# mit-han-lab/qserve

Hardware: NVIDIA H100
Metric: tokens/s Llama-3-8B W4A8KV4 decode b64 (higher is better)
Workload: dtype s8

## Files before the change

qserve_b200/csrc/gemm.cu:

```cuda
#include <cstdarg>
#include <cstdio>
#include <cstdlib>
#include <cstring>
#include <mutex>
#include <unordered_map>

#include "common.cuh"
#include "launch.cuh"

namespace qs {

namespace {

constexpr int kBM = 128;
constexpr int kBK = 128;
constexpr int kSub = 2;
constexpr int kConsumers = 128;
constexpr int kNumThreads = 192;
constexpr int kFrag = 4;

enum { kModeW4Chn = 0, kModeW4Grp = 1, kModeW8 = 2 };

struct GemmParams {
  const uint8_t* s2_scales;
  const uint8_t* s2_zeros;
  const __half* wscales;
  const __half* w_szs;
  const __half* ascales;
  const __half* a_ssums;
  __half* out;
  int32_t* acc_out;
  int M, N, K;
  int m_tiles, kb_per_tile, split;
  unsigned long long* prof;
};

template <int MODE, int NT, int WS, int AS>
struct Cfg {
  static constexpr int kActSub = NT * kBK;
  static constexpr int kWSub = (MODE == kModeW8) ? kBM * kBK : kBM * kBK / 2;
  static constexpr int kS2Sub = (MODE == kModeW4Grp) ? 2 * kBM : 0;
  static constexpr int kActBytes = kSub * kActSub;
  static constexpr int kWBytes = kSub * kWSub;
  static constexpr int kS2Bytes = kSub * kS2Sub;
  static constexpr int kWStageTx = kWBytes + kS2Bytes;
  static constexpr int kOffAct = 0;
  static constexpr int kOffW = kOffAct + AS * kActBytes;
  static constexpr int kOffS2 = kOffW + WS * kWBytes;
  static constexpr int kPipeBytes = kOffS2 + WS * kS2Bytes;
  static constexpr int kRedBytes = NT * kBM * 4;
  static constexpr int kOffRow = (kPipeBytes > kRedBytes ? kPipeBytes : kRedBytes);
  static constexpr int kOffBar = kOffRow + 2 * NT * 4;
  static constexpr int kNumBars = 2 * WS + 2 * AS;
  static constexpr int kSmemBytes = kOffBar + kNumBars * 8;
  static constexpr int kCtasPerSm = (NT <= 64 && kSmemBytes <= 113 * 1024) ? 2 : 1;
  static_assert(kSmemBytes <= 227 * 1024, "shared memory overflow");
};

__device__ __forceinline__ unsigned long long gtime() {
  unsigned long long t;
  asm volatile("mov.u64 %0, %globaltimer;" : "=l"(t)::"memory");
  return t;
}
#define QS_PROF(slot) do { if (p.prof) p.prof[blockIdx.x * 16 + (slot)] = gtime(); } while (0)

__device__ __forceinline__ uint32_t cluster_ctarank() {
  uint32_t r;
  asm volatile("mov.u32 %0, %%cluster_ctarank;" : "=r"(r));
  return r;
}
__device__ __forceinline__ void cluster_sync_all() {
  asm volatile("barrier.cluster.arrive.release.aligned;\n\tbarrier.cluster.wait.acquire.aligned;" ::: "memory");
}
__device__ __forceinline__ void cluster_arrive() { asm volatile("barrier.cluster.arrive.release;" ::: "memory"); }
__device__ __forceinline__ void cluster_wait() { asm volatile("barrier.cluster.wait.acquire;" ::: "memory"); }
__device__ __forceinline__ uint32_t smid() {
  uint32_t r;
  asm volatile("mov.u32 %0, %%smid;" : "=r"(r));
  return r;
}
__device__ __forceinline__ uint32_t map_to_cta(uint32_t smem_addr, uint32_t rank) {
  uint32_t r;
  asm volatile("mapa.shared::cluster.u32 %0, %1, %2;" : "=r"(r) : "r"(smem_addr), "r"(rank));
  return r;
}
__device__ __forceinline__ void st_dsmem_u32(uint32_t addr, uint32_t v) {
  asm volatile("st.shared::cluster.u32 [%0], %1;" ::"r"(addr), "r"(v) : "memory");
}

template <int V>
struct IntTag { static constexpr int value = V; };

template <int MODE>
__device__ __forceinline__ float epilogue_one(int32_t acc, float ws, float wsz, float as, float asum) {
  float ps = __int2float_rn(acc);
  if constexpr (MODE == kModeW4Chn) {
    float t = __fmul_rn(__fmul_rn(ps, ws), as);
    float u = __fmul_rn(wsz, asum);
    return __fsub_rn(t, u);
  } else {
    return __fmul_rn(ps, __fmul_rn(ws, as));
  }
}

template <int MODE>
__device__ __forceinline__ int acc_channel(int h, int w, int r) {
  return (MODE == kModeW8) ? 64 * h + 16 * w + r : 32 * w + 16 * h + r;
}

template <int MODE, int NT, int WS, int AS, bool ACC>
__global__ void __launch_bounds__(kNumThreads, Cfg<MODE, NT, WS, AS>::kCtasPerSm)
gemm_kernel(const __grid_constant__ CUtensorMap tmap_act, const __grid_constant__ CUtensorMap tmap_w, const GemmParams p) {
  using C = Cfg<MODE, NT, WS, AS>;
  extern __shared__ __align__(1024) uint8_t smem[];
  if (threadIdx.x == 0 && (smem_u32(smem) & 1023u) != 0) __trap();
  uint8_t* s_act = smem + C::kOffAct;
  uint8_t* s_w = smem + C::kOffW;
  uint8_t* s_s2 = smem + C::kOffS2;
  int32_t* s_red = reinterpret_cast<int32_t*>(smem);
  float* s_asc = reinterpret_cast<float*>(smem + C::kOffRow);
  float* s_asum = s_asc + NT;
  uint64_t* bar_wfull = reinterpret_cast<uint64_t*>(smem + C::kOffBar);
  uint64_t* bar_wempty = bar_wfull + WS;
  uint64_t* bar_xfull = bar_wempty + WS;
  uint64_t* bar_xempty = bar_xfull + AS;

  const int warp = threadIdx.x >> 5;
  const int lane = threadIdx.x & 31;
  const int S = p.split;
  const int rank = (S > 1) ? static_cast<int>(cluster_ctarank()) : 0;
  const int tile = blockIdx.x / S;
  const int m_tile = tile % p.m_tiles, n_tile = tile / p.m_tiles;
  const int KB = p.kb_per_tile;
  const int kb_begin = (KB * rank) / S, kb_end = (KB * (rank + 1)) / S;
  const int n_kb = kb_end - kb_begin;
  if (threadIdx.x == 0) {
    QS_PROF(0);
    if (p.prof) p.prof[blockIdx.x * 16 + 15] = smid();
  }
  qs_trace(QS_K_GEMM, 0);

  if (threadIdx.x == 0) {
    tma_prefetch_desc(&tmap_act);
    tma_prefetch_desc(&tmap_w);
    for (int i = 0; i < WS; ++i) {
      mbar_init(&bar_wfull[i], 1);
      mbar_init(&bar_wempty[i], 4);
    }
    for (int i = 0; i < AS; ++i) {
      mbar_init(&bar_xfull[i], 1);
      mbar_init(&bar_xempty[i], 4);
    }
    fence_barrier_init();
  }
  __syncthreads();
  if (threadIdx.x == 0) { pdl_launch_dependents(); QS_PROF(1); }

  if (warp == 4) {
    if (lane == 0) {
      const int w_row = (MODE == kModeW8) ? n_tile * kBM : n_tile * 4;
      const uint8_t* s2s = p.s2_scales + static_cast<size_t>(n_tile) * kBM;
      const uint8_t* s2z = p.s2_zeros + static_cast<size_t>(n_tile) * kBM;
      int s = 0;
      uint32_t ph = 0;
      for (int it = 0; it < n_kb; ++it) {
        if (it >= WS) mbar_wait_nocall(&bar_wempty[s], ph);
        mbar_expect_tx(&bar_wfull[s], C::kWStageTx);
#pragma unroll
        for (int u = 0; u < kSub; ++u) {
          const int kb = (kb_begin + it) * kSub + u;
          tma_load_2d(s_w + s * C::kWBytes + u * C::kWSub, &tmap_w, (MODE == kModeW8) ? kb * kBK : kb * 256, w_row, &bar_wfull[s]);
          if constexpr (MODE == kModeW4Grp) {
            const int kg = kb < p.K / kBK ? kb : p.K / kBK - 1;
            bulk_copy_g2s(s_s2 + s * C::kS2Bytes + u * C::kS2Sub, s2s + static_cast<size_t>(kg) * p.N, kBM, &bar_wfull[s]);
            bulk_copy_g2s(s_s2 + s * C::kS2Bytes + u * C::kS2Sub + kBM, s2z + static_cast<size_t>(kg) * p.N, kBM, &bar_wfull[s]);
          }
        }
        if (++s == WS) { s = 0; if (it >= WS) ph ^= 1; }
      }
      QS_PROF(3);
    }
  } else if (warp == 5) {
    if (lane == 0) {
      const int a_row = m_tile * NT;
      pdl_wait();
      QS_PROF(2);
      qs_trace(QS_K_GEMM, 1, 5 * 32);
      int s = 0;
      uint32_t ph = 0;
      for (int it = 0; it < n_kb; ++it) {
        if (it >= AS) mbar_wait_nocall(&bar_xempty[s], ph);
        mbar_expect_tx(&bar_xfull[s], C::kActBytes);
#pragma unroll
        for (int u = 0; u < kSub; ++u)
          tma_load_2d(s_act + s * C::kActBytes + u * C::kActSub, &tmap_act, ((kb_begin + it) * kSub + u) * kBK, a_row, &bar_xfull[s]);
        if (++s == AS) { s = 0; if (it >= AS) ph ^= 1; }
      }
    }
  } else {
    int32_t acc[2][NT / 2];
#pragma unroll
    for (int h = 0; h < 2; ++h)
#pragma unroll
      for (int i = 0; i < NT / 2; ++i) acc[h][i] = 0;
    mbar_wait_nocall(&bar_wfull[0], 0);
    mbar_wait_nocall(&bar_xfull[0], 0);
    if (threadIdx.x == 0) QS_PROF(4);
    const bool leader = lane == 0;
    int sw = 0, sx = 0, prev_sw = WS - 1, prev_sx = AS - 1;
    uint32_t phw = 0, phx = 0;
    for (int it = 0; it < n_kb; ++it) {
      mbar_wait_nocall(&bar_wfull[sw], phw);
      mbar_wait_nocall(&bar_xfull[sx], phx);
      if constexpr (MODE == kModeW8) {
#pragma unroll
        for (int u = 0; u < kSub; ++u) {
          const uint64_t bdesc = gmma_desc_sw128(smem_u32(s_act + sx * C::kActBytes + u * C::kActSub));
          const uint64_t adesc = gmma_desc_sw128(smem_u32(s_w + sw * C::kWBytes + u * C::kWSub));
          wgmma_fence();
#pragma unroll
          for (int t = 0; t < kBK / 32; ++t) {
            wgmma_s8_ss(acc[0], adesc + t * 2, bdesc + t * 2);
            wgmma_s8_ss(acc[1], adesc + (64 * kBK >> 4) + t * 2, bdesc + t * 2);
          }
          wgmma_commit();
        }
        wgmma_wait<kSub>();
        mbar_arrive_if(&bar_wempty[prev_sw], it > 0 && leader);
        mbar_arrive_if(&bar_xempty[prev_sx], it > 0 && leader);
      } else {
        uint32_t fr[kFrag][2][4];
#pragma unroll
        for (int u = 0; u < kSub; ++u) {
          const uint64_t bdesc = gmma_desc_sw128(smem_u32(s_act + sx * C::kActBytes + u * C::kActSub));
          const uint8_t* wsrc = s_w + sw * C::kWBytes + u * C::kWSub + warp * 2048 + lane * 16;
          uint32_t sc4 = 0, zp4 = 0;
          if constexpr (MODE == kModeW4Grp) {
            const uint8_t* s2 = s_s2 + sw * C::kS2Bytes + u * C::kS2Sub + warp * 32 + (lane >> 2) * 4;
            sc4 = *reinterpret_cast<const uint32_t*>(s2);
            zp4 = *reinterpret_cast<const uint32_t*>(s2 + kBM);
          }
#pragma unroll
          for (int t = 0; t < 4; ++t) {
            const int j = u * 4 + t;
            const uint4 v = *reinterpret_cast<const uint4*>(wsrc + t * 512);
            uint32_t xl = v.x & 0x0F0F0F0Fu, xh = (v.x >> 4) & 0x0F0F0F0Fu;
            uint32_t yl = v.y & 0x0F0F0F0Fu, yh = (v.y >> 4) & 0x0F0F0F0Fu;
            uint32_t zl = v.z & 0x0F0F0F0Fu, zh = (v.z >> 4) & 0x0F0F0F0Fu;
            uint32_t wl = v.w & 0x0F0F0F0Fu, wh = (v.w >> 4) & 0x0F0F0F0Fu;
            if constexpr (MODE == kModeW4Grp) {
              const uint32_t s0 = sc4 & 0xFF, s1 = (sc4 >> 8) & 0xFF, s2 = (sc4 >> 16) & 0xFF, s3 = sc4 >> 24;
              const uint32_t z0 = __byte_perm(zp4, 0, 0x0000), z1 = __byte_perm(zp4, 0, 0x1111);
              const uint32_t z2 = __byte_perm(zp4, 0, 0x2222), z3 = __byte_perm(zp4, 0, 0x3333);
              xl = __vadd4(xl * s0, z0); zl = __vadd4(zl * s0, z0);
              yl = __vadd4(yl * s1, z1); wl = __vadd4(wl * s1, z1);
              xh = __vadd4(xh * s2, z2); zh = __vadd4(zh * s2, z2);
              yh = __vadd4(yh * s3, z3); wh = __vadd4(wh * s3, z3);
            }
            wgmma_wait<kFrag - 1>();
            if (j == kFrag - 1) mbar_arrive_if(&bar_xempty[prev_sx], it > 0 && leader);
            uint32_t(&f)[2][4] = fr[j % kFrag];
            f[0][0] = xl; f[0][1] = yl; f[0][2] = zl; f[0][3] = wl;
            f[1][0] = xh; f[1][1] = yh; f[1][2] = zh; f[1][3] = wh;
            wgmma_fence();
            wgmma_s8_rs(acc[0], f[0], bdesc + t * 2);
            wgmma_s8_rs(acc[1], f[1], bdesc + t * 2);
            wgmma_commit();
          }
        }
        mbar_arrive_if(&bar_wempty[sw], leader);
      }
      prev_sw = sw;
      prev_sx = sx;
      if (++sw == WS) { sw = 0; phw ^= 1; }
      if (++sx == AS) { sx = 0; phx ^= 1; }
    }
    wgmma_wait<0>();
    if (threadIdx.x == 0) QS_PROF(6);
    if (S > 1) cluster_arrive();

    const int epi_tid = threadIdx.x;
    pdl_wait();
    const int m0 = m_tile * NT;
    for (int j = epi_tid; j < NT; j += kConsumers) {
      const bool ok = (m0 + j) < p.M;
      s_asc[j] = ok ? __half2float(p.ascales[m0 + j]) : 0.f;
      if constexpr (MODE == kModeW4Chn) s_asum[j] = ok ? __half2float(p.a_ssums[m0 + j]) : 0.f;
    }
    if (S > 1) cluster_wait(); else named_bar_sync(1, kConsumers);
    if (epi_tid == 0) QS_PROF(8);
    const int r0 = lane >> 2, c0 = (lane & 3) * 2;
    if (S == 1) {
#pragma unroll
      for (int h = 0; h < 2; ++h)
#pragma unroll
        for (int i = 0; i < NT / 2; ++i) {
          const int ch = acc_channel<MODE>(h, warp, r0 + 8 * ((i >> 1) & 1));
          const int tok = (i >> 2) * 8 + c0 + (i & 1);
          s_red[tok * kBM + ch] = acc[h][i];
        }
    } else {
      const int cps = kBM / S;
      const uint32_t rx_base = smem_u32(s_red);
#pragma unroll
      for (int h = 0; h < 2; ++h)
#pragma unroll
        for (int i = 0; i < NT / 2; ++i) {
          const int ch = acc_channel<MODE>(h, warp, r0 + 8 * ((i >> 1) & 1));
          const int tok = (i >> 2) * 8 + c0 + (i & 1);
          const uint32_t owner = static_cast<uint32_t>(ch / cps);
          st_dsmem_u32(map_to_cta(rx_base, owner) + static_cast<uint32_t>(((rank * NT + tok) * cps + ch % cps) * 4), static_cast<uint32_t>(acc[h][i]));
        }
    }
    if (epi_tid == 0) QS_PROF(9);
  }
  if (S > 1 && threadIdx.x >= kConsumers) { cluster_arrive(); cluster_wait(); }

  if (S > 1) cluster_sync_all(); else __syncthreads();
  if (threadIdx.x < kConsumers) {
    pdl_wait();
    const int tid = threadIdx.x;
    if (tid == 0) QS_PROF(10);
    const int npairs = 64 / S;
    const int pr = (64 * rank) / S + tid % npairs;
    const float ws0 = __half2float(__ldg(p.wscales + n_tile * kBM + 2 * pr)), ws1 = __half2float(__ldg(p.wscales + n_tile * kBM + 2 * pr + 1));
    float wz0 = 0.f, wz1 = 0.f;
    if constexpr (MODE == kModeW4Chn) {
      wz0 = __half2float(__ldg(p.w_szs + n_tile * kBM + 2 * pr));
      wz1 = __half2float(__ldg(p.w_szs + n_tile * kBM + 2 * pr + 1));
    }
    const int m0 = m_tile * NT;
    const int tstep = kConsumers / npairs;
    const int n = n_tile * kBM + 2 * pr;
    const int tok_end = min(NT, p.M - m0);
    const int tok0 = tid / npairs;
    const uint32_t off0 = static_cast<uint32_t>((tok0 * kBM + 2 * pr) * 4), off_step = static_cast<uint32_t>(tstep * kBM * 4);
    __half* optr = p.out + static_cast<size_t>(m0 + tok0) * p.N + n;
    const size_t ostep = static_cast<size_t>(tstep) * p.N;
    auto finish = [&](int tok, int2 acc, __half* dst) {
      const float as = s_asc[tok], asum = s_asum[tok];
      const float o0 = epilogue_one<MODE>(acc.x, ws0, wz0, as, asum);
      const float o1 = epilogue_one<MODE>(acc.y, ws1, wz1, as, asum);
      *reinterpret_cast<__half2*>(dst) = __floats2half2_rn(o0, o1);
      if constexpr (ACC) *reinterpret_cast<int2*>(p.acc_out + (dst - p.out)) = acc;
    };
    if (S == 1) {
      constexpr int kPerThread = NT / 2;
#pragma unroll 1
      for (int i0 = 0; i0 < kPerThread; i0 += 16) {
        int2 v[16];
#pragma unroll
        for (int e = 0; e < 16; ++e)
          if (kPerThread > e) v[e] = *reinterpret_cast<const int2*>(reinterpret_cast<const uint8_t*>(s_red) + off0 + (i0 + e) * off_step);
#pragma unroll
        for (int e = 0; e < 16; ++e) {
          const int tok = tok0 + (i0 + e) * tstep;
          if (kPerThread > e && tok < tok_end) finish(tok, v[e], optr + (i0 + e) * ostep);
        }
      }
    } else {
      const int cps = kBM / S;
      const int32_t* rx = s_red;
      const int prl = tid % npairs;
      auto reduce_rows = [&](auto s_tag) {
        constexpr int SS = decltype(s_tag)::value;
        constexpr int TPT = NT / (2 * SS) > 0 ? NT / (2 * SS) : 1;
        int2 v[TPT][SS];
#pragma unroll
        for (int i = 0; i < TPT; ++i) {
          const int tok = tok0 + i * tstep;
#pragma unroll
          for (int r = 0; r < SS; ++r)
            v[i][r] = (tok < NT) ? *reinterpret_cast<const int2*>(rx + (r * NT + tok) * cps + 2 * prl) : make_int2(0, 0);
        }
#pragma unroll
        for (int i = 0; i < TPT; ++i) {
          const int tok = tok0 + i * tstep;
          int2 acc = v[i][0];
#pragma unroll
          for (int r = 1; r < SS; ++r) { acc.x += v[i][r].x; acc.y += v[i][r].y; }
          if (tok < tok_end) finish(tok, acc, optr + i * ostep);
        }
      };
      if (S == 2) reduce_rows(IntTag<2>{});
      else if (S == 4) reduce_rows(IntTag<4>{});
      else reduce_rows(IntTag<8>{});
    }
    if (tid == 0) QS_PROF(11);
  } else {
    pdl_wait();
  }
  if (threadIdx.x == 0) QS_PROF(12);
  qs_trace(QS_K_GEMM, 2);
}


struct TmapKey {
  const void* ptr; uint64_t a, b; uint32_t box, kind;
  bool operator==(const TmapKey& o) const { return ptr == o.ptr && a == o.a && b == o.b && box == o.box && kind == o.kind; }
};
struct TmapKeyHash {
  size_t operator()(const TmapKey& k) const {
    size_t h = reinterpret_cast<size_t>(k.ptr) * 0x9E3779B97F4A7C15ull;
    h ^= (k.a + 0x7F4A7C15ull + (h << 6) + (h >> 2));
    h ^= (k.b * 0xC2B2AE3D27D4EB4Full + (h << 6) + (h >> 2));
    return h ^ (static_cast<size_t>(k.box) << 7) ^ k.kind;
  }
};
std::unordered_map<TmapKey, CUtensorMap, TmapKeyHash>& tmap_cache() {
  static std::unordered_map<TmapKey, CUtensorMap, TmapKeyHash> c;
  return c;
}
std::mutex& tmap_mutex() { static std::mutex m; return m; }
bool tmap_lookup(const TmapKey& k, CUtensorMap* m) {
  std::lock_guard<std::mutex> g(tmap_mutex());
  auto it = tmap_cache().find(k);
  if (it == tmap_cache().end()) return false;
  memcpy(m, &it->second, sizeof(CUtensorMap));
  return true;
}
void tmap_store(const TmapKey& k, const CUtensorMap* m) {
  std::lock_guard<std::mutex> g(tmap_mutex());
  if (tmap_cache().size() > 16384) tmap_cache().clear();
  memcpy(&tmap_cache()[k], m, sizeof(CUtensorMap));
}

int make_tmap_u8(CUtensorMap* m, const void* ptr, uint64_t rows, uint64_t cols, uint32_t box_rows) {
  const TmapKey key{ptr, rows, cols, box_rows, 0u};
  if (tmap_lookup(key, m)) return QS_OK;
  PFN_encodeTiled enc = get_encode();
  if (!enc) return set_error(QS_ERR_CUDA, "cuTensorMapEncodeTiled entry point not available");
  cuuint64_t dims[2] = {cols, rows};
  cuuint64_t strides[1] = {cols};
  cuuint32_t box[2] = {128, box_rows};
  cuuint32_t estr[2] = {1, 1};
  CUresult r = enc(m, CU_TENSOR_MAP_DATA_TYPE_UINT8, 2, const_cast<void*>(ptr), dims, strides, box, estr, CU_TENSOR_MAP_INTERLEAVE_NONE,
                   CU_TENSOR_MAP_SWIZZLE_128B, CU_TENSOR_MAP_L2_PROMOTION_L2_256B, CU_TENSOR_MAP_FLOAT_OOB_FILL_NONE);
  if (r != CUDA_SUCCESS) return set_error(QS_ERR_CUDA, "cuTensorMapEncodeTiled failed (%d): ptr=%p rows=%llu cols=%llu box_rows=%u", (int)r, ptr,
                                          (unsigned long long)rows, (unsigned long long)cols, box_rows);
  tmap_store(key, m);
  return QS_OK;
}

int make_tmap_w4(CUtensorMap* m, const void* ptr, uint64_t N, uint64_t K, uint32_t box_bands = 4) {
  const TmapKey key{ptr, N, K, box_bands, 1u};
  if (tmap_lookup(key, m)) return QS_OK;
  PFN_encodeTiled enc = get_encode();
  if (!enc) return set_error(QS_ERR_CUDA, "cuTensorMapEncodeTiled entry point not available");
  cuuint64_t dims[2] = {K * 16 / 8, N / 32};
  cuuint64_t strides[1] = {K * 16};
  cuuint32_t box[2] = {256, box_bands};
  cuuint32_t estr[2] = {1, 1};
  CUresult r = enc(m, CU_TENSOR_MAP_DATA_TYPE_INT64, 2, const_cast<void*>(ptr), dims, strides, box, estr, CU_TENSOR_MAP_INTERLEAVE_NONE,
                   CU_TENSOR_MAP_SWIZZLE_NONE, CU_TENSOR_MAP_L2_PROMOTION_L2_256B, CU_TENSOR_MAP_FLOAT_OOB_FILL_NONE);
  if (r != CUDA_SUCCESS) return set_error(QS_ERR_CUDA, "cuTensorMapEncodeTiled(w4) failed (%d): ptr=%p N=%llu K=%llu", (int)r, ptr, (unsigned long long)N,
                                          (unsigned long long)K);
  tmap_store(key, m);
  return QS_OK;
}

int resident_clusters(const void* kern, int smem, int s) {
  int n = 0;
  if (s == 1) {
    if (cudaOccupancyMaxActiveBlocksPerMultiprocessor(&n, kern, kNumThreads, smem) != cudaSuccess) n = 0;
    return n * num_sms();
  }
  cudaLaunchConfig_t cfg{};
  cfg.gridDim = dim3(s);
  cfg.blockDim = dim3(kNumThreads);
  cfg.dynamicSmemBytes = smem;
  cudaLaunchAttribute attr;
  attr.id = cudaLaunchAttributeClusterDimension;
  attr.val.clusterDim.x = s;
  attr.val.clusterDim.y = 1;
  attr.val.clusterDim.z = 1;
  cfg.attrs = &attr;
  cfg.numAttrs = 1;
  if (cudaOccupancyMaxActiveClusters(&n, kern, &cfg) != cudaSuccess) n = 0;
  return n;
}

template <typename Resident>
int choose_split(int tiles, int kb_per_tile, int forced, Resident resident) {
  int s = 1;
  if (forced > 0) {
    s = forced;
  } else {
    while (s < 8 && kb_per_tile >= 4 * s && tiles <= resident(2 * s)) s *= 2;
  }
  while (s > 1 && kb_per_tile < s) s /= 2;
  return s;
}

template <int MODE, int NT, int WS, int AS>
int launch_gemm(const GemmArgs& a) {
  using C = Cfg<MODE, NT, WS, AS>;
  GemmParams p{};
  p.s2_scales = static_cast<const uint8_t*>(a.s2_scales);
  p.s2_zeros = static_cast<const uint8_t*>(a.s2_zeros);
  p.wscales = static_cast<const __half*>(a.wscales);
  p.w_szs = static_cast<const __half*>(a.w_szs);
  p.ascales = static_cast<const __half*>(a.ascales);
  p.a_ssums = static_cast<const __half*>(a.a_ssums);
  p.out = static_cast<__half*>(a.out);
  p.acc_out = static_cast<int32_t*>(a.acc_out);
  p.prof = static_cast<unsigned long long*>(a.prof);
  p.M = a.M; p.N = a.N; p.K = a.K;
  const int n_tiles = a.N / kBM;
  p.m_tiles = (a.M + NT - 1) / NT;
  p.kb_per_tile = (a.K + kSub * kBK - 1) / (kSub * kBK);
  const int tiles = n_tiles * p.m_tiles;

  CUtensorMap tm_act, tm_w;
  int rc = make_tmap_u8(&tm_act, a.act, a.M, a.K, NT);
  if (rc) return rc;
  rc = (MODE == kModeW8) ? make_tmap_u8(&tm_w, a.weight, a.N, a.K, kBM) : make_tmap_w4(&tm_w, a.weight, a.N, a.K);
  if (rc) return rc;

  auto kern = a.acc_out ? gemm_kernel<MODE, NT, WS, AS, true> : gemm_kernel<MODE, NT, WS, AS, false>;
  rc = raise_smem_limit(kern, C::kSmemBytes, "cudaFuncSetAttribute(gemm smem)");
  if (rc) return rc;
  const int dev = device_ordinal();
  static int resident_cache[2][kMaxDevices][4] = {};
  auto resident = [&](int s) {
    int& r = resident_cache[a.acc_out ? 1 : 0][dev][s == 1 ? 0 : s == 2 ? 1 : s == 4 ? 2 : 3];
    if (r == 0) r = resident_clusters(reinterpret_cast<const void*>(kern), C::kSmemBytes, s);
    return r;
  };
  p.split = choose_split(tiles, p.kb_per_tile, a.force_split, resident);
  if (p.prof)
    fprintf(stderr, "qs_gemm_plan mode=%d nt=%d ws=%d as=%d M=%d N=%d K=%d tiles=%d split=%d ctas=%d smem=%d resident_clusters=%d\n", MODE, NT, WS,
            AS, a.M, a.N, a.K, tiles, p.split, tiles * p.split, C::kSmemBytes, resident(p.split));
  return launch(kern, dim3(tiles * p.split), dim3(kNumThreads), C::kSmemBytes, p.split, a.stream, "gemm launch", tm_act, tm_w, p);
}

template <int MODE>
int dispatch_gemm(const GemmArgs& a) {
  QS_REQUIRE(a.M > 0 && a.N > 0 && a.K > 0, "gemm: empty problem M=%d N=%d K=%d", a.M, a.N, a.K);
  QS_REQUIRE(a.N % kBM == 0, "gemm: N=%d must be a multiple of %d", a.N, kBM);
  QS_REQUIRE(a.K % kBK == 0, "gemm: K=%d must be a multiple of %d", a.K, kBK);
  QS_REQUIRE((reinterpret_cast<uintptr_t>(a.act) & 15) == 0 && (reinterpret_cast<uintptr_t>(a.weight) & 15) == 0, "gemm: operands must be 16-byte aligned");
  QS_REQUIRE(a.force_split == 0 || a.force_split == 1 || a.force_split == 2 || a.force_split == 4 || a.force_split == 8, "gemm: split must be 1, 2, 4 or 8");
  constexpr bool w8 = (MODE == kModeW8), grp = (MODE == kModeW4Grp);
  QS_REQUIRE(a.force_nt == 0 || a.force_nt == 32 || a.force_nt == 64 || a.force_nt == 128, "gemm: tile tokens must be 32, 64 or 128");
  const int nt = a.force_nt > 0 ? a.force_nt : a.M <= 32 ? 32 : a.M <= 64 ? 64 : 128;
  if (nt == 32) return launch_gemm<MODE, 32, (w8 ? 2 : grp ? 4 : 5), 4>(a);
  if (nt == 64) return launch_gemm<MODE, 64, (w8 ? 2 : grp ? 3 : 4), (w8 ? 2 : 3)>(a);
  return launch_gemm<MODE, 128, 4, 2>(a);
}

}

int gemm_w4a8_per_chn(const GemmArgs& a) { return dispatch_gemm<kModeW4Chn>(a); }
int gemm_w4a8_per_group(const GemmArgs& a) { return dispatch_gemm<kModeW4Grp>(a); }
int gemm_w8a8(const GemmArgs& a) { return dispatch_gemm<kModeW8>(a); }
size_t gemm_workspace_bytes() { return 4096; }
int gemm_trace_install(void* buf, unsigned cap) { return qs_trace_install(buf, cap); }

}
```

Before: 14470.

## Use bulk DSMEM copies for split-K reduction and cost-based tile/split planning

Split-K partial sums are first staged locally in a swizzled layout. They are then pushed to peer CTAs with cp.async.bulk shared::cluster copies that complete on an mbarrier, replacing per-element st.shared::cluster stores and a full cluster sync. The S==1 and S>1 epilogues are unified, and the weight-scale loads are hoisted before pdl_wait. The dispatcher now searches over tile-token sizes and split factors that fit in residency, minimising the number of K stages per CTA, where before the tile size was fixed by M and the split chosen greedily. This may pick smaller token tiles and larger splits, which re-reads weights more often.

New measurement: 15020 (median of 6 runs). 1.04x the previous value.

```diff
diff --git a/qserve_b200/csrc/gemm.cu b/qserve_b200/csrc/gemm.cu
--- a/qserve_b200/csrc/gemm.cu
+++ b/qserve_b200/csrc/gemm.cu
@@ -49,9 +49,11 @@
   static constexpr int kOffS2 = kOffW + WS * kWBytes;
   static constexpr int kPipeBytes = kOffS2 + WS * kS2Bytes;
   static constexpr int kRedBytes = NT * kBM * 4;
+  static constexpr int kOffTx = kRedBytes;
+  static_assert(2 * kRedBytes <= kPipeBytes, "receive and staging buffer must both fit in the drained rings");
   static constexpr int kOffRow = (kPipeBytes > kRedBytes ? kPipeBytes : kRedBytes);
   static constexpr int kOffBar = kOffRow + 2 * NT * 4;
-  static constexpr int kNumBars = 2 * WS + 2 * AS;
+  static constexpr int kNumBars = 2 * WS + 2 * AS + 1;
   static constexpr int kSmemBytes = kOffBar + kNumBars * 8;
   static constexpr int kCtasPerSm = (NT <= 64 && kSmemBytes <= 113 * 1024) ? 2 : 1;
   static_assert(kSmemBytes <= 227 * 1024, "shared memory overflow");
@@ -68,9 +70,6 @@
   uint32_t r;
   asm volatile("mov.u32 %0, %%cluster_ctarank;" : "=r"(r));
   return r;
-}
-__device__ __forceinline__ void cluster_sync_all() {
-  asm volatile("barrier.cluster.arrive.release.aligned;\n\tbarrier.cluster.wait.acquire.aligned;" ::: "memory");
 }
 __device__ __forceinline__ void cluster_arrive() { asm volatile("barrier.cluster.arrive.release;" ::: "memory"); }
 __device__ __forceinline__ void cluster_wait() { asm volatile("barrier.cluster.wait.acquire;" ::: "memory"); }
@@ -84,9 +83,11 @@
   asm volatile("mapa.shared::cluster.u32 %0, %1, %2;" : "=r"(r) : "r"(smem_addr), "r"(rank));
   return r;
 }
-__device__ __forceinline__ void st_dsmem_u32(uint32_t addr, uint32_t v) {
-  asm volatile("st.shared::cluster.u32 [%0], %1;" ::"r"(addr), "r"(v) : "memory");
-}
+__device__ __forceinline__ void bulk_copy_s2peer(uint32_t dst, uint32_t src, uint32_t bytes, uint32_t bar) {
+  asm volatile("cp.async.bulk.shared::cluster.shared::cta.mbarrier::complete_tx::bytes [%0], [%1], %2, [%3];" ::"r"(dst), "r"(src), "r"(bytes), "r"(bar)
+               : "memory");
+}
+__device__ __forceinline__ int red_swizzle(int tok, int width) { return (((tok >> 1) & 3) << 3) & (width - 1); }
 
 template <int V>
 struct IntTag { static constexpr int value = V; };
@@ -124,6 +125,7 @@
   uint64_t* bar_wempty = bar_wfull + WS;
   uint64_t* bar_xfull = bar_wempty + WS;
   uint64_t* bar_xempty = bar_xfull + AS;
+  uint64_t* bar_red = bar_xempty + AS;
 
   const int warp = threadIdx.x >> 5;
   const int lane = threadIdx.x & 31;
@@ -136,7 +138,11 @@
   const int n_kb = kb_end - kb_begin;
   if (threadIdx.x == 0) {
     QS_PROF(0);
-    if (p.prof) p.prof[blockIdx.x * 16 + 15] = smid();
+    if (p.prof) {
+      p.prof[blockIdx.x * 16 + 13] = NT;
+      p.prof[blockIdx.x * 16 + 14] = S;
+      p.prof[blockIdx.x * 16 + 15] = smid();
+    }
   }
   qs_trace(QS_K_GEMM, 0);
 
@@ -151,6 +157,8 @@
       mbar_init(&bar_xfull[i], 1);
       mbar_init(&bar_xempty[i], 4);
     }
+    mbar_init(bar_red, 1);
+    if (S > 1) mbar_expect_tx(bar_red, static_cast<uint32_t>((S - 1) * NT * (kBM / S) * 4));
     fence_barrier_init();
   }
   __syncthreads();
@@ -279,62 +287,59 @@
     if (threadIdx.x == 0) QS_PROF(6);
     if (S > 1) cluster_arrive();
 
-    const int epi_tid = threadIdx.x;
+    named_bar_sync(1, kConsumers);
+    const int tid = threadIdx.x;
+    const int cps_log2 = 8 - __ffs(S), cps = 1 << cps_log2;
+    int32_t* s_tx = s_red + (S > 1 ? C::kOffTx / 4 : 0);
+    {
+      const int r0 = lane >> 2, c0 = (lane & 3) * 2;
+#pragma unroll
+      for (int h = 0; h < 2; ++h)
+#pragma unroll
+        for (int i = 0; i < NT / 2; ++i) {
+          const int ch = acc_channel<MODE>(h, warp, r0 + 8 * ((i >> 1) & 1));
+          const int tok = (i >> 2) * 8 + c0 + (i & 1);
+          s_tx[(((ch >> cps_log2) * NT + tok) << cps_log2) + ((ch & (cps - 1)) ^ red_swizzle(tok, cps))] = acc[h][i];
+        }
+    }
+    const int npairs = 64 / S;
+    const int prl = tid % npairs;
+    const int n = n_tile * kBM + 2 * ((64 * rank) / S + prl);
+    const float ws0 = __half2float(__ldg(p.wscales + n)), ws1 = __half2float(__ldg(p.wscales + n + 1));
+    float wz0 = 0.f, wz1 = 0.f;
+    if constexpr (MODE == kModeW4Chn) {
+      wz0 = __half2float(__ldg(p.w_szs + n));
+      wz1 = __half2float(__ldg(p.w_szs + n + 1));
+    }
     pdl_wait();
     const int m0 = m_tile * NT;
-    for (int j = epi_tid; j < NT; j += kConsumers) {
+    for (int j = tid; j < NT; j += kConsumers) {
       const bool ok = (m0 + j) < p.M;
       s_asc[j] = ok ? __half2float(p.ascales[m0 + j]) : 0.f;
       if constexpr (MODE == kModeW4Chn) s_asum[j] = ok ? __half2float(p.a_ssums[m0 + j]) : 0.f;
     }
-    if (S > 1) cluster_wait(); else named_bar_sync(1, kConsumers);
-    if (epi_tid == 0) QS_PROF(8);
-    const int r0 = lane >> 2, c0 = (lane & 3) * 2;
-    if (S == 1) {
-#pragma unroll
-      for (int h = 0; h < 2; ++h)
-#pragma unroll
-        for (int i = 0; i < NT / 2; ++i) {
-          const int ch = acc_channel<MODE>(h, warp, r0 + 8 * ((i >> 1) & 1));
-          const int tok = (i >> 2) * 8 + c0 + (i & 1);
-          s_red[tok * kBM + ch] = acc[h][i];
-        }
-    } else {
-      const int cps = kBM / S;
-      const uint32_t rx_base = smem_u32(s_red);
-#pragma unroll
-      for (int h = 0; h < 2; ++h)
-#pragma unroll
-        for (int i = 0; i < NT / 2; ++i) {
-          const int ch = acc_channel<MODE>(h, warp, r0 + 8 * ((i >> 1) & 1));
-          const int tok = (i >> 2) * 8 + c0 + (i & 1);
-          const uint32_t owner = static_cast<uint32_t>(ch / cps);
-          st_dsmem_u32(map_to_cta(rx_base, owner) + static_cast<uint32_t>(((rank * NT + tok) * cps + ch % cps) * 4), static_cast<uint32_t>(acc[h][i]));
-        }
-    }
-    if (epi_tid == 0) QS_PROF(9);
-  }
-  if (S > 1 && threadIdx.x >= kConsumers) { cluster_arrive(); cluster_wait(); }
-
-  if (S > 1) cluster_sync_all(); else __syncthreads();
-  if (threadIdx.x < kConsumers) {
-    pdl_wait();
-    const int tid = threadIdx.x;
+    if (S > 1) {
+      fence_proxy_async();
+      cluster_wait();
+    }
+    if (tid == 0) QS_PROF(8);
+    named_bar_sync(1, kConsumers);
+    if (S > 1) {
+      if (tid < S && tid != rank) {
+        const uint32_t slice = static_cast<uint32_t>(NT * cps * 4);
+        bulk_copy_s2peer(map_to_cta(smem_u32(s_red) + rank * slice, tid), smem_u32(s_tx) + tid * slice, slice, map_to_cta(smem_u32(bar_red), tid));
+      }
+      if (tid == 0) QS_PROF(9);
+      mbar_wait_nocall(bar_red, 0);
+      cluster_arrive();
+    } else if (tid == 0) {
+      QS_PROF(9);
+    }
     if (tid == 0) QS_PROF(10);
-    const int npairs = 64 / S;
-    const int pr = (64 * rank) / S + tid % npairs;
-    const float ws0 = __half2float(__ldg(p.wscales + n_tile * kBM + 2 * pr)), ws1 = __half2float(__ldg(p.wscales + n_tile * kBM + 2 * pr + 1));
-    float wz0 = 0.f, wz1 = 0.f;
-    if constexpr (MODE == kModeW4Chn) {
-      wz0 = __half2float(__ldg(p.w_szs + n_tile * kBM + 2 * pr));
-      wz1 = __half2float(__ldg(p.w_szs + n_tile * kBM + 2 * pr + 1));
-    }
-    const int m0 = m_tile * NT;
+
     const int tstep = kConsumers / npairs;
-    const int n = n_tile * kBM + 2 * pr;
     const int tok_end = min(NT, p.M - m0);
     const int tok0 = tid / npairs;
-    const uint32_t off0 = static_cast<uint32_t>((tok0 * kBM + 2 * pr) * 4), off_step = static_cast<uint32_t>(tstep * kBM * 4);
     __half* optr = p.out + static_cast<size_t>(m0 + tok0) * p.N + n;
     const size_t ostep = static_cast<size_t>(tstep) * p.N;
     auto finish = [&](int tok, int2 acc, __half* dst) {
@@ -344,54 +349,51 @@
       *reinterpret_cast<__half2*>(dst) = __floats2half2_rn(o0, o1);
       if constexpr (ACC) *reinterpret_cast<int2*>(p.acc_out + (dst - p.out)) = acc;
     };
-    if (S == 1) {
-      constexpr int kPerThread = NT / 2;
+    auto reduce_rows = [&](auto s_tag) {
+      constexpr int SS = decltype(s_tag)::value;
+      constexpr int CPS = kBM / SS;
+      constexpr int TPT = NT / (2 * SS) > 0 ? NT / (2 * SS) : 1;
+      constexpr int kChunk = TPT * SS > 16 ? 16 / SS : TPT;
 #pragma unroll 1
-      for (int i0 = 0; i0 < kPerThread; i0 += 16) {
-        int2 v[16];
-#pragma unroll
-        for (int e = 0; e < 16; ++e)
-          if (kPerThread > e) v[e] = *reinterpret_cast<const int2*>(reinterpret_cast<const uint8_t*>(s_red) + off0 + (i0 + e) * off_step);
-#pragma unroll
-        for (int e = 0; e < 16; ++e) {
-          const int tok = tok0 + (i0 + e) * tstep;
-          if (kPerThread > e && tok < tok_end) finish(tok, v[e], optr + (i0 + e) * ostep);
+      for (int i0 = 0; i0 < TPT; i0 += kChunk) {
+        int2 v[kChunk][SS];
+#pragma unroll
+        for (int i = 0; i < kChunk; ++i) {
+          const int tok = tok0 + (i0 + i) * tstep;
+#pragma unroll
+          for (int r = 0; r < SS; ++r) {
+            const int32_t* src = (SS > 1 && r != rank) ? s_red + r * NT * CPS : s_tx + rank * NT * CPS;
+            v[i][r] = (tok < NT) ? *reinterpret_cast<const int2*>(src + tok * CPS + ((2 * prl) ^ red_swizzle(tok, CPS))) : make_int2(0, 0);
+          }
+        }
+#pragma unroll
+        for (int i = 0; i < kChunk; ++i) {
+          const int tok = tok0 + (i0 + i) * tstep;
+          int2 acc = v[i][0];
+#pragma unroll
+          for (int r = 1; r < SS; ++r) { acc.x += v[i][r].x; acc.y += v[i][r].y; }
+          if (tok < tok_end) finish(tok, acc, optr + (i0 + i) * ostep);
         }
       }
-    } else {
-      const int cps = kBM / S;
-      const int32_t* rx = s_red;
-      const int prl = tid % npairs;
-      auto reduce_rows = [&](auto s_tag) {
-        constexpr int SS = decltype(s_tag)::value;
-        constexpr int TPT = NT / (2 * SS) > 0 ? NT / (2 * SS) : 1;
-        int2 v[TPT][SS];
-#pragma unroll
-        for (int i = 0; i < TPT; ++i) {
-          const int tok = tok0 + i * tstep;
-#pragma unroll
-          for (int r = 0; r < SS; ++r)
-            v[i][r] = (tok < NT) ? *reinterpret_cast<const int2*>(rx + (r * NT + tok) * cps + 2 * prl) : make_int2(0, 0);
-        }
-#pragma unroll
-        for (int i = 0; i < TPT; ++i) {
-          const int tok = tok0 + i * tstep;
-          int2 acc = v[i][0];
-#pragma unroll
-          for (int r = 1; r < SS; ++r) { acc.x += v[i][r].x; acc.y += v[i][r].y; }
-          if (tok < tok_end) finish(tok, acc, optr + i * ostep);
-        }
-      };
-      if (S == 2) reduce_rows(IntTag<2>{});
-      else if (S == 4) reduce_rows(IntTag<4>{});
-      else reduce_rows(IntTag<8>{});
-    }
+    };
+    if (S == 1) reduce_rows(IntTag<1>{});
+    else if (S == 2) reduce_rows(IntTag<2>{});
+    else if (S == 4) reduce_rows(IntTag<4>{});
+    else reduce_rows(IntTag<8>{});
     if (tid == 0) QS_PROF(11);
-  } else {
-    pdl_wait();
-  }
-  if (threadIdx.x == 0) QS_PROF(12);
-  qs_trace(QS_K_GEMM, 2);
+    if (S > 1) cluster_wait();
+    if (tid == 0) QS_PROF(12);
+    qs_trace(QS_K_GEMM, 2);
+    return;
+  }
+  if (S > 1) {
+    cluster_arrive();
+    cluster_wait();
+    cluster_arrive();
+    cluster_wait();
+  }
+  __syncwarp();
+  pdl_wait();
 }
 
 
@@ -480,20 +482,19 @@
   return n;
 }
 
-template <typename Resident>
-int choose_split(int tiles, int kb_per_tile, int forced, Resident resident) {
-  int s = 1;
-  if (forced > 0) {
-    s = forced;
-  } else {
-    while (s < 8 && kb_per_tile >= 4 * s && tiles <= resident(2 * s)) s *= 2;
-  }
-  while (s > 1 && kb_per_tile < s) s /= 2;
-  return s;
-}
-
 template <int MODE, int NT, int WS, int AS>
-int launch_gemm(const GemmArgs& a) {
+int resident_gemm(const GemmArgs& a, int s) {
+  using C = Cfg<MODE, NT, WS, AS>;
+  auto kern = a.acc_out ? gemm_kernel<MODE, NT, WS, AS, true> : gemm_kernel<MODE, NT, WS, AS, false>;
+  static int cache[2][kMaxDevices][4] = {};
+  int& r = cache[a.acc_out ? 1 : 0][device_ordinal()][s == 1 ? 0 : s == 2 ? 1 : s == 4 ? 2 : 3];
+  if (r == 0 && raise_smem_limit(kern, C::kSmemBytes, "cudaFuncSetAttribute(gemm smem)") == QS_OK)
+    r = resident_clusters(reinterpret_cast<const void*>(kern), C::kSmemBytes, s);
+  return r;
+}
+
+template <int MODE, int NT, int WS, int AS>
+int launch_gemm(const GemmArgs& a, int split) {
   using C = Cfg<MODE, NT, WS, AS>;
   GemmParams p{};
   p.s2_scales = static_cast<const uint8_t*>(a.s2_scales);
@@ -520,19 +521,20 @@
   auto kern = a.acc_out ? gemm_kernel<MODE, NT, WS, AS, true> : gemm_kernel<MODE, NT, WS, AS, false>;
   rc = raise_smem_limit(kern, C::kSmemBytes, "cudaFuncSetAttribute(gemm smem)");
   if (rc) return rc;
-  const int dev = device_ordinal();
-  static int resident_cache[2][kMaxDevices][4] = {};
-  auto resident = [&](int s) {
-    int& r = resident_cache[a.acc_out ? 1 : 0][dev][s == 1 ? 0 : s == 2 ? 1 : s == 4 ? 2 : 3];
-    if (r == 0) r = resident_clusters(reinterpret_cast<const void*>(kern), C::kSmemBytes, s);
-    return r;
-  };
-  p.split = choose_split(tiles, p.kb_per_tile, a.force_split, resident);
+  p.split = split;
   if (p.prof)
     fprintf(stderr, "qs_gemm_plan mode=%d nt=%d ws=%d as=%d M=%d N=%d K=%d tiles=%d split=%d ctas=%d smem=%d resident_clusters=%d\n", MODE, NT, WS,
-            AS, a.M, a.N, a.K, tiles, p.split, tiles * p.split, C::kSmemBytes, resident(p.split));
+            AS, a.M, a.N, a.K, tiles, p.split, tiles * p.split, C::kSmemBytes, resident_gemm<MODE, NT, WS, AS>(a, p.split));
   return launch(kern, dim3(tiles * p.split), dim3(kNumThreads), C::kSmemBytes, p.split, a.stream, "gemm launch", tm_act, tm_w, p);
 }
+
+struct TileImpl {
+  int nt;
+  int (*resident)(const GemmArgs&, int);
+  int (*launch)(const GemmArgs&, int);
+};
+
+inline long plan_cost(int nt, int s, int stages) { return stages * 1000L + (128 - nt) + s; }
 
 template <int MODE>
 int dispatch_gemm(const GemmArgs& a) {
@@ -541,12 +543,34 @@
   QS_REQUIRE(a.K % kBK == 0, "gemm: K=%d must be a multiple of %d", a.K, kBK);
   QS_REQUIRE((reinterpret_cast<uintptr_t>(a.act) & 15) == 0 && (reinterpret_cast<uintptr_t>(a.weight) & 15) == 0, "gemm: operands must be 16-byte aligned");
   QS_REQUIRE(a.force_split == 0 || a.force_split == 1 || a.force_split == 2 || a.force_split == 4 || a.force_split == 8, "gemm: split must be 1, 2, 4 or 8");
+  QS_REQUIRE(a.force_nt == 0 || a.force_nt == 32 || a.force_nt == 64 || a.force_nt == 128, "gemm: tile tokens must be 32, 64 or 128");
   constexpr bool w8 = (MODE == kModeW8), grp = (MODE == kModeW4Grp);
-  QS_REQUIRE(a.force_nt == 0 || a.force_nt == 32 || a.force_nt == 64 || a.force_nt == 128, "gemm: tile tokens must be 32, 64 or 128");
-  const int nt = a.force_nt > 0 ? a.force_nt : a.M <= 32 ? 32 : a.M <= 64 ? 64 : 128;
-  if (nt == 32) return launch_gemm<MODE, 32, (w8 ? 2 : grp ? 4 : 5), 4>(a);
-  if (nt == 64) return launch_gemm<MODE, 64, (w8 ? 2 : grp ? 3 : 4), (w8 ? 2 : 3)>(a);
-  return launch_gemm<MODE, 128, 4, 2>(a);
+  constexpr int kWs32 = w8 ? 2 : grp ? 4 : 5, kWs64 = w8 ? 2 : grp ? 3 : 4, kAs64 = w8 ? 2 : 3;
+  static const TileImpl impls[3] = {{32, resident_gemm<MODE, 32, kWs32, 4>, launch_gemm<MODE, 32, kWs32, 4>},
+                                    {64, resident_gemm<MODE, 64, kWs64, kAs64>, launch_gemm<MODE, 64, kWs64, kAs64>},
+                                    {128, resident_gemm<MODE, 128, 4, 2>, launch_gemm<MODE, 128, 4, 2>}};
+  const int kb = (a.K + kSub * kBK - 1) / (kSub * kBK);
+  const int nt_cover = a.M <= 32 ? 32 : a.M <= 64 ? 64 : 128;
+  int forced_s = a.force_split;
+  while (forced_s > 1 && kb < forced_s) forced_s /= 2;
+  const TileImpl* best = nullptr;
+  int best_s = 0;
+  long best_cost = 0;
+  for (const TileImpl& t : impls) {
+    if (a.force_nt > 0 ? t.nt != a.force_nt : t.nt > nt_cover) continue;
+    const int tiles = (a.N / kBM) * ((a.M + t.nt - 1) / t.nt);
+    for (int s = 1; s <= 8; s *= 2) {
+      if (forced_s > 0 ? s != forced_s : (s > 1 && kb < 2 * s)) continue;
+      if (tiles > t.resident(a, s)) continue;
+      const long cost = plan_cost(t.nt, s, (kb + s - 1) / s);
+      if (best == nullptr || cost < best_cost) best = &t, best_s = s, best_cost = cost;
+    }
+  }
+  if (best == nullptr) {
+    best = &impls[(a.force_nt > 0 ? a.force_nt : nt_cover) == 32 ? 0 : (a.force_nt > 0 ? a.force_nt : nt_cover) == 64 ? 1 : 2];
+    best_s = forced_s > 0 ? forced_s : 1;
+  }
+  return best->launch(a, best_s);
 }
 
 }
```
